# CityU-AIM-Group/SCAN

Measured on AMD Instinct MI355X. Metric: train images/sec (whole node), VGG16 C2F 1024x2048, higher is better.
Workload: dtype f32 (fp32 storage, fp32 multiply, fp32 accumulate -- the reference's arithmetic; the convolutions run it on the bf16 matrix cores as bf16x6: every fp32 operand cut into 3 bf16 pieces = all 24 significand bits, 6 bf16 MFMAs per product)

## Files before the change

### scan_amd/csrc/capi.cpp

```cpp
#include <stdarg.h>
#include <stdio.h>
#include <string.h>

#include "../../include/scan_hip.h"
#include "conv_launch.h"

static thread_local char g_err[512] = "";

extern "C" void scan_set_error(const char* fmt, ...) {
  va_list ap;
  va_start(ap, fmt);
  vsnprintf(g_err, sizeof(g_err), fmt, ap);
  va_end(ap);
}

extern "C" const char* scan_last_error(void) { return g_err; }
extern "C" int scan_abi_version(void) { return 1; }

int g_scan_deterministic = 0;

struct Knob {
  const char* key;
  int* slot;
  int dflt;
};
static Knob* knob_table(int* count) {
  static Knob knobs[] = {
      {"conv_bn256", &g_scan_conv_bn256, 0},   {"conv_v2", &g_scan_conv_v2, 0},         {"conv_wg1024", &g_scan_conv_wg1024, 0},
      {"conv_w8", &g_scan_conv_w8, 0},         {"conv_tpb3", &g_scan_conv_tpb3, 0},     {"conv_bn64_th16", &g_scan_conv_bn64_th16, 0},
      {"conv_glds", &g_scan_conv_glds, 0},     {"wgrad_v6", &g_scan_wgrad_v6, 0},       {"wgrad_prio", &g_scan_wgrad_prio, 0},
      {"wgrad_tile", &g_scan_wgrad_tile, 0},   {"wgrad_wgs", &g_scan_wgrad_wgs, 0},     {"gconv_mfma", &g_scan_gconv_mfma, 0},
      {"dbscan_bf16x3", &g_scan_dbscan_bf16x3, 0}, {"reduce_blocks", &g_scan_reduce_blocks, 0}, {"conv1x1", &g_scan_conv1x1, 0},
      {"conv_wino", &g_scan_conv_wino, 0},     {"wgrad_wino", &g_scan_wgrad_wino, 0},   {"wino_tpb", &g_scan_wino_tpb, 0},
      {"deterministic", &g_scan_deterministic, 0}, {"dynconv_generic", &g_scan_dynconv_generic, 0},
  };
  static bool init = false;
  if (!init) {
    for (auto& k : knobs) k.dflt = *k.slot;
    init = true;
  }
  *count = (int)(sizeof(knobs) / sizeof(knobs[0]));
  return knobs;
}
static Knob* find_knob(const char* key) {
  int n = 0;
  Knob* t = knob_table(&n);
  if (key == nullptr) return nullptr;
  for (int i = 0; i < n; ++i)
    if (strcmp(key, t[i].key) == 0) return &t[i];
  return nullptr;
}

extern "C" int scan_tune(const char* key, int value) {
  Knob* k = find_knob(key);
  if (k == nullptr) return SCAN_TUNE_UNKNOWN;
  const int old = *k->slot;
  *k->slot = value;
  return old;
}

extern "C" int scan_tune_get(const char* key) {
  const Knob* k = find_knob(key);
  return k == nullptr ? SCAN_TUNE_UNKNOWN : *k->slot;
}

extern "C" int scan_tune_default(const char* key) {
  const Knob* k = find_knob(key);
  return k == nullptr ? SCAN_TUNE_UNKNOWN : k->dflt;
}

extern "C" const char* scan_tune_key(int index) {
  int n = 0;
  const Knob* t = knob_table(&n);
  return (index >= 0 && index < n) ? t[index].key : nullptr;
}
```

### scan_amd/csrc/conv_fwd.hip

```cpp
#include "conv_launch.h"
#include "conv_split.h"

#define V2_TW CONV_TILE_W
#ifndef SCAN_CONV_MID
#define SCAN_CONV_MID 0
#endif
#ifndef SCAN_CONV_PFA
#define SCAN_CONV_PFA 1
#endif
#define V2_CK 32

__device__ __forceinline__ int swz(int idx) { return (idx >> 1) & 2; }
__device__ __forceinline__ int wsw(int t, int r) { return ((t >> 1) & 2) ^ (r & 1); }

template <int V>
struct IntC {
  static constexpr int value = V;
};

template <int K>
__device__ __forceinline__ const __bf16* pick_plane(const __bf16* w0, const __bf16* w1, const __bf16* w2) {
  if constexpr (K == 0)
    return w0;
  else if constexpr (K == 1)
    return w1;
  else
    return w2;
}
template <int I, int NT, int PL, int NPL>
__device__ __forceinline__ const __bf16* slot_plane(int tid, const __bf16* w0, const __bf16* w1, const __bf16* w2) {
  constexpr int lo = (NT * I) / PL, hi = (NT * I + NT - 1) / PL;
  constexpr int lo_c = lo < NPL ? lo : NPL - 1, hi_c = hi < NPL ? hi : NPL - 1;
  static_assert(hi - lo <= 1, "a thread's slot spans at most two planes");
  if constexpr (lo_c == hi_c)
    return pick_plane<lo_c>(w0, w1, w2);
  else
    return (tid + NT * I) / PL == lo ? pick_plane<lo_c>(w0, w1, w2) : pick_plane<hi_c>(w0, w1, w2);
}
template <int NT, int PL, int NPL>
__device__ __forceinline__ const __bf16* slot_plane_i(int i, int tid, const __bf16* w0, const __bf16* w1, const __bf16* w2) {
  return i == 0   ? slot_plane<0, NT, PL, NPL>(tid, w0, w1, w2)
         : i == 1 ? slot_plane<1, NT, PL, NPL>(tid, w0, w1, w2)
         : i == 2 ? slot_plane<2, NT, PL, NPL>(tid, w0, w1, w2)
         : i == 3 ? slot_plane<3, NT, PL, NPL>(tid, w0, w1, w2)
         : i == 4 ? slot_plane<4, NT, PL, NPL>(tid, w0, w1, w2)
                  : slot_plane<5, NT, PL, NPL>(tid, w0, w1, w2);
}

template <int NP, int TM, bool TEMP = false>
__device__ __forceinline__ void mma_pieces(const bf16x8 (&w)[NP], const bf16x8 (&p)[NP][TM], f32x4v (&acc)[TM]) {
  if constexpr (TEMP) {
    f32x4v t[TM];
#pragma unroll
    for (int tm = 0; tm < TM; ++tm) t[tm] = f32x4v{0.f, 0.f, 0.f, 0.f};
#pragma unroll
    for (int s = NP - 1; s >= 0; --s)
#pragma unroll
      for (int i = 0; i <= s; ++i)
#pragma unroll
        for (int tm = 0; tm < TM; ++tm) t[tm] = __builtin_amdgcn_mfma_f32_16x16x32_bf16(w[i], p[s - i][tm], t[tm], 0, 0, 0);
#pragma unroll
    for (int tm = 0; tm < TM; ++tm) acc[tm] += t[tm];
    return;
  }
#pragma unroll
  for (int s = NP - 1; s >= 0; --s)
#pragma unroll
    for (int i = 0; i <= s; ++i)
#pragma unroll
      for (int tm = 0; tm < TM; ++tm) acc[tm] = __builtin_amdgcn_mfma_f32_16x16x32_bf16(w[i], p[s - i][tm], acc[tm], 0, 0, 0);
}

__device__ __forceinline__ void gn_sums_add(const float4 o, double& ds, double& dq) {
  const double o0 = (double)o.x, o1 = (double)o.y, o2 = (double)o.z, o3 = (double)o.w;
  ds += (o0 + o1) + (o2 + o3);
  dq += (o0 * o0 + o1 * o1) + (o2 * o2 + o3 * o3);
}

template <int NP, int BN, int TH, int NT, int KS, int TPB = 1, bool GL = false, bool WINO = false>
__global__ __launch_bounds__(NT, NT == 1024 ? 4 : 2) void conv_split_kernel(
    const float* __restrict__ src, scan_pyramid_t d, int Cs, const __bf16* __restrict__ w0, const __bf16* __restrict__ w1,
    const __bf16* __restrict__ w2, int Csw, const float* __restrict__ bias, const float* __restrict__ mask,
    float* __restrict__ dst, int Nout, int Ns, int relu, TileTab2 tt, int n_tiles, scan_pyramid_t sd, int map,
    double* __restrict__ gn_ws) {
  constexpr int HALO = KS / 2, NTAPS = KS * KS;
  constexpr int PH = TH + 2 * HALO;
  constexpr int WJ = WINO ? (TPB == 2 ? 2 : 4) : 1;
  constexpr int PWK = WINO ? WJ * 8 : V2_TW + 2 * HALO;
  constexpr int NPATCH = PH * PWK;
  constexpr int WTAPS = WINO ? 12 : NTAPS;
  constexpr int WAVES = NT / 64;
  constexpr int WN_WAVES = BN >= 128 ? 2 : 1;
  constexpr int WM_WAVES = WAVES / WN_WAVES;
  constexpr int TM = TH / WM_WAVES;
  constexpr int TN = BN / (16 * WN_WAVES);
  constexpr int TMW = WINO ? TM / 2 : TM;
  constexpr int ASLOTS = WINO ? (PH * 64 + NT - 1) / NT : (NPATCH * 8 + NT - 1) / NT;
  constexpr int AK = WINO ? 4 : 1;
  constexpr int BSLOTS = BN * 4 * NP;
  constexpr int BSEG = (BSLOTS + NT - 1) / NT;
  constexpr int NGRP = WTAPS / TPB;
  static_assert(NP == 2 || NP == 3, "two or three pieces per operand");
  static_assert(TM * WM_WAVES == TH && (TM % 2) == 0, "tile rows must split evenly (and pair up for the fused pool)");
  static_assert(WTAPS % TPB == 0, "taps per barrier must divide the tap count");
  static_assert(BSLOTS % 64 == 0, "a wave's 64 weight segments lie in one plane (and past the end only as a whole wave)");
  static_assert(!WINO || (GL && KS == 3 && (TPB == 1 || TPB == 2) && NP == 3 && TM % 2 == 0), "Winograd: three pieces, 3x3, LDS-DMA weights");

  extern __shared__ __align__(16) unsigned char smem_raw[];
  __bf16* As = reinterpret_cast<__bf16*>(smem_raw);
  __bf16* Bs = As + NP * NPATCH * 32;

  const int tid = threadIdx.x, lane = tid & 63, wid = tid >> 6;
  const int bid = xcd_remap(blockIdx.x, gridDim.x);
  const int n_tile = bid % n_tiles;
  const int tile = bid / n_tiles;
  int lvl = 0;
#pragma unroll
  for (int i = 1; i < SCAN_MAX_LEVELS; ++i)
    if (i < d.n_levels && tile >= tt.tile_off[i]) lvl = i;
  const int H = d.h[lvl], W = d.w[lvl];
  int t = tile - tt.tile_off[lvl];
  const int per_img = tt.tiles_x[lvl] * tt.tiles_y[lvl];
  const int img = t / per_img;
  t -= img * per_img;
  const int ty0 = (t / tt.tiles_x[lvl]) * TH, tx0 = (t % tt.tiles_x[lvl]) * V2_TW;
  const int64_t rowbase = d.row_off[lvl] + (int64_t)img * H * W;
  const int n0 = n_tile * BN;
  const int nchunks = (Cs + V2_CK - 1) / V2_CK;

  constexpr unsigned BAD = 0x80000000u;
  unsigned voff[ASLOTS];
  unsigned vok = 0;
  const int c_tail = Cs - (nchunks - 1) * V2_CK;
  const bool tail_bad = 4 * (tid & 7) >= c_tail;
  __amdgpu_buffer_rsrc_t a_src;
  {
    const bool mapped = KS == 1 && map != 0;
    const int Hs = mapped ? sd.h[lvl] : H, Ws = mapped ? sd.w[lvl] : W;
    int64_t base_row;
    if (!mapped)
      base_row = rowbase + (int64_t)(ty0 - HALO) * W + (tx0 - HALO);
    else if (map == 1)
      base_row = sd.row_off[lvl] + ((int64_t)img * Hs + 2 * ty0) * Ws + 2 * tx0;
    else
      base_row = sd.row_off[lvl] + ((int64_t)img * Hs + (ty0 >> 1)) * Ws + (tx0 >> 1);
    a_src = uniform_rsrc_b(src + base_row * Cs, 0x7ffffff0);
    if constexpr (WINO) {
#pragma unroll
      for (int i = 0; i < ASLOTS; ++i) {
        const int slot = tid + NT * i;
        const int c4 = slot & 7, t = (slot >> 3) & 7, py = slot >> 6;
        voff[i] = (unsigned)(((py * W + 2 * t) * Cs + 4 * c4) * 4);
#pragma unroll
        for (int k = 0; k < 4; ++k) {
          const int y = ty0 - HALO + py, x = tx0 - HALO + 2 * t + k;
          if ((slot < PH * 64) && y >= 0 && y < H && x >= 0 && x < W) vok |= 1u << (4 * i + k);
        }
      }
    } else {
#pragma unroll
      for (int i = 0; i < ASLOTS; ++i) {
        const int slot = tid + NT * i;
        const int q = slot >> 3, c4 = slot & 7;
        const int py = q / PWK, px = q - py * PWK;
        const int y = ty0 - HALO + py, x = tx0 - HALO + px;
        bool ok = (slot < NPATCH * 8) && y >= 0 && y < H && x >= 0 && x < W;
        int pix = py * W + px;
        if (mapped) {
          if (map == 1) {
            ok = ok && 2 * y < Hs && 2 * x < Ws;
            pix = 2 * py * Ws + 2 * px;
          } else {
            ok = ok && ((y | x) & 1) == 0 && (y >> 1) < Hs && (x >> 1) < Ws;
            pix = (py >> 1) * Ws + (px >> 1);
          }
        }
        voff[i] = ok ? (unsigned)((pix * Cs + 4 * c4) * 4) : BAD;
      }
    }
  }
  float4 ra[ASLOTS][AK];
  auto load_a = [&](int cc) {
    const int soff = cc * (V2_CK * 4);
    const bool kill = tail_bad && cc == nchunks - 1;
    if constexpr (WINO && TPB == 2) {
      unsigned vk = vok;
      asm volatile("" : "+v"(vk));
#pragma unroll
      for (int i = 0; i < ASLOTS; ++i)
#pragma unroll
        for (int k = 0; k < AK; ++k) {
          const bool ok = ((vk >> (4 * i + k)) & 1) && !kill;
          ra[i][k] = __builtin_bit_cast(float4, __builtin_amdgcn_raw_buffer_load_b128(a_src, (int)(ok ? voff[0] : BAD),
                                                                                      soff + (i * (NT / 64) * W + k) * Cs * 4, 0));
        }
      return;
    }
#pragma unroll
    for (int i = 0; i < ASLOTS; ++i)
#pragma unroll
      for (int k = 0; k < AK; ++k) {
        const unsigned off = !WINO ? voff[i] : ((vok >> (4 * i + k)) & 1) ? voff[i] + (unsigned)(k * Cs * 4) : BAD;
        ra[i][k] = __builtin_bit_cast(float4, __builtin_amdgcn_raw_buffer_load_b128(a_src, (int)(kill ? BAD : off), soff, 0));
      }
  };
  auto store_a = [&](auto half_c) {
    if constexpr (WINO) {
      constexpr int half = decltype(half_c)::value;
#pragma unroll
      for (int i = 0; i < ASLOTS; ++i) {
        const int slot = tid + NT * i;
        if (slot < PH * 64) {
          const int c4 = slot & 7, t = (slot >> 3) & 7, py = slot >> 6;
          const float4 d0 = ra[i][0], d1 = ra[i][1], d2 = ra[i][2], d3 = ra[i][3];
          const float4 u[4] = {make_float4(d0.x - d2.x, d0.y - d2.y, d0.z - d2.z, d0.w - d2.w),
                               make_float4(d1.x + d2.x, d1.y + d2.y, d1.z + d2.z, d1.w + d2.w),
                               make_float4(d2.x - d1.x, d2.y - d1.y, d2.z - d1.z, d2.w - d1.w),
                               make_float4(d1.x - d3.x, d1.y - d3.y, d1.z - d3.z, d1.w - d3.w)};
          const int sl = (((c4 >> 1) ^ wsw(t, py)) << 3) + ((c4 & 1) << 2);
#pragma unroll
          for (int j = 0; j < WJ; ++j) {
            bf16x4 pc[NP];
            split4_np<NP>(u[WJ == 4 ? j : 2 * half + j], pc);
            const int off = (py * PWK + j * 8 + t) * 32 + sl;
#pragma unroll
            for (int p = 0; p < NP; ++p) *reinterpret_cast<bf16x4*>(As + p * NPATCH * 32 + off) = pc[p];
          }
        }
      }
      return;
    }
#pragma unroll
    for (int i = 0; i < ASLOTS; ++i) {
      const int slot = tid + NT * i;
      if (slot < NPATCH * 8) {
        const int q = slot >> 3, c4 = slot & 7;
        const int px = q % PWK;
        bf16x4 pc[NP];
        split4_np<NP>(ra[i][0], pc);
        const int off = q * 32 + (((c4 >> 1) ^ swz(px)) << 3) + ((c4 & 1) << 2);
#pragma unroll
        for (int p = 0; p < NP; ++p) *reinterpret_cast<bf16x4*>(As + p * NPATCH * 32 + off) = pc[p];
      }
    }
  };
  uint4 rb[TPB][BSEG];
  auto load_b = [&](int cc, int grp) {
#pragma unroll
    for (int tt = 0; tt < TPB; ++tt) {
      const int tap = grp * TPB + tt;
#pragma unroll
      for (int i = 0; i < BSEG; ++i) {
        const int slot = tid + NT * i;
        const int plane = slot / (BN * 4);
        const int rem = slot - plane * BN * 4;
        const int row = rem >> 2, seg = rem & 3;
        const int o = n0 + row, c = cc * V2_CK + 8 * seg;
        const __bf16* base = slot_plane_i<NT, BN * 4, NP>(i, tid, w0, w1, w2);
        rb[tt][i] = (slot < BSLOTS && o < Nout && c < Csw)
                        ? *reinterpret_cast<const uint4*>(base + ((int64_t)o * NTAPS + tap) * Csw + c)
                        : make_uint4(0u, 0u, 0u, 0u);
      }
    }
  };
  auto store_b = [&](int buf) {
#pragma unroll
    for (int tt = 0; tt < TPB; ++tt) {
#pragma unroll
      for (int i = 0; i < BSEG; ++i) {
        const int slot = tid + NT * i;
        const int plane = slot / (BN * 4);
        const int rem = slot - plane * BN * 4;
        const int row = rem >> 2, seg = rem & 3;
        if (slot < BSLOTS)
          *reinterpret_cast<uint4*>(Bs + (((buf * TPB + tt) * NP + plane) * BN + row) * 32 + ((seg ^ swz(row)) << 3)) = rb[tt][i];
      }
    }
  };

  static_assert(!GL || BSEG <= 6, "the LDS-DMA path keeps at most six descriptors");
  unsigned boff[BSEG];
#pragma unroll
  for (int i = 0; i < BSEG; ++i) {
    const int slot = tid + NT * i;
    const int plane = slot / (BN * 4);
    const int rem = slot - plane * BN * 4;
    const int row = rem >> 2, seg = (rem & 3) ^ swz(row);
    boff[i] = (unsigned)((((n0 + row) * WTAPS) * Csw + 8 * seg) * 2);
  }
  const int plane_bytes = Nout * WTAPS * Csw * 2;
  auto plane_rsrc = [&](int i) { return uniform_rsrc_b(slot_plane_i<NT, BN * 4, NP>(i, tid, w0, w1, w2), plane_bytes); };
  const __amdgpu_buffer_rsrc_t b_src0 = plane_rsrc(0), b_src1 = plane_rsrc(1), b_src2 = plane_rsrc(2),
                               b_src3 = plane_rsrc(3), b_src4 = plane_rsrc(4), b_src5 = plane_rsrc(5);
  auto issue_b = [&](int cc, int grp, int buf) {
#pragma unroll
    for (int tt = 0; tt < TPB; ++tt) {
      const int tap = grp * TPB + tt;
      const int soff = (tap * Csw + cc * V2_CK) * 2;
#pragma unroll
      for (int i = 0; i < BSEG; ++i) {
        const int slot = tid + NT * i;
        if (BSEG * NT != BSLOTS && slot - lane >= BSLOTS) continue;
        const int plane = slot / (BN * 4);
        const int rem = slot - plane * BN * 4;
        __bf16* dst_l = Bs + (((buf * TPB + tt) * NP + plane) * BN) * 32 + (rem - lane) * 8;
        __builtin_amdgcn_raw_ptr_buffer_load_lds(
            i == 0 ? b_src0 : i == 1 ? b_src1 : i == 2 ? b_src2 : i == 3 ? b_src3 : i == 4 ? b_src4 : b_src5, (lds_ptr_t)dst_l,
            16, (int)boff[i], soff, 0, 0);
      }
    }
  };

  const int wm = wid / WN_WAVES, wn = wid % WN_WAVES;
  const int lr = lane & 15, kg = lane >> 4;
  const int w_row0 = wn * 16 * TN + lr;
  const int w_off = w_row0 * 32 + ((kg ^ swz(w_row0)) << 3);

  f32x4v acc[TN][TM];
#pragma unroll
  for (int b = 0; b < TN; ++b)
#pragma unroll
    for (int a = 0; a < TM; ++a) acc[b][a] = f32x4v{0.f, 0.f, 0.f, 0.f};
  f32x4v wacc[WINO ? 4 : 1][WINO ? TN : 1][TMW];
#pragma unroll
  for (int j = 0; j < (WINO ? 4 : 1); ++j)
#pragma unroll
    for (int b = 0; b < (WINO ? TN : 1); ++b)
#pragma unroll
      for (int a = 0; a < TMW; ++a) wacc[j][b][a] = f32x4v{0.f, 0.f, 0.f, 0.f};

  auto patch_off = [&](int tap) {
    const int ky = tap / KS, kx = tap - KS * ky;
    const int pxs = lr + kx;
    return ((wm * TM + ky) * PWK + pxs) * 32 + ((kg ^ swz(pxs)) << 3);
  };
  auto read_patch = [&](int tap, bf16x8 (&pf)[NP][TM]) {
    const int p_off = patch_off(tap);
#pragma unroll
    for (int p = 0; p < NP; ++p)
#pragma unroll
      for (int tm = 0; tm < TM; ++tm)
        pf[p][tm] = *reinterpret_cast<const bf16x8*>(As + p * NPATCH * 32 + p_off + tm * PWK * 32);
  };
  auto read_w = [&](const __bf16* bt, int tn, bf16x8 (&wf)[NP]) {
#pragma unroll
    for (int p = 0; p < NP; ++p) wf[p] = *reinterpret_cast<const bf16x8*>(bt + p * BN * 32 + tn * 16 * 32);
  };
  auto taps_mma = [&](int grp, int buf, auto&& mid) {
#pragma unroll
    for (int tt = 0; tt < TPB; ++tt) {
      const int tap = grp * TPB + tt;
      const __bf16* bt = Bs + ((buf * TPB + tt) * NP) * BN * 32 + w_off;
      bf16x8 pf[NP][TM];
      read_patch(tap, pf);
#pragma unroll
      for (int tn = 0; tn < TN; ++tn) {
        bf16x8 wf[NP];
        read_w(bt, tn, wf);
        mma_pieces<NP, TM, KS == 1 && NP == 3>(wf, pf, acc[tn]);
        if (tt == 0 && tn == SCAN_CONV_MID) {
          __builtin_amdgcn_sched_barrier(0);
          mid();
          __builtin_amdgcn_sched_barrier(0);
        }
      }
    }
  };
  auto no_mid = []() {};

  constexpr bool PFA = GL && NT == 512 && TPB == 1 && NP == 2 && SCAN_CONV_PFA;
  bf16x8 npf[NP][TM];
  auto taps_mma_pf = [&](int grp, int buf, auto&& mid) {
    if constexpr (PFA) {
      const __bf16* bt = Bs + (buf * NP) * BN * 32 + w_off;
      if (grp == 0) read_patch(0, npf);
#pragma unroll
      for (int tn = 0; tn < TN - 1; ++tn) {
        bf16x8 wf[NP];
        read_w(bt, tn, wf);
        mma_pieces<NP, TM>(wf, npf, acc[tn]);
        if (tn == SCAN_CONV_MID) {
          __builtin_amdgcn_sched_barrier(0);
          mid();
          __builtin_amdgcn_sched_barrier(0);
        }
      }
      {
        constexpr int tn = TN - 1;
        bf16x8 wf[NP];
        read_w(bt, tn, wf);
        const bool more = grp < NGRP - 1;
        const int p_off = patch_off(more ? grp + 1 : grp);
#pragma unroll
        for (int tm = 0; tm < TM; ++tm) {
          acc[tn][tm] = __builtin_amdgcn_mfma_f32_16x16x32_bf16(wf[0], npf[1][tm], acc[tn][tm], 0, 0, 0);
          acc[tn][tm] = __builtin_amdgcn_mfma_f32_16x16x32_bf16(wf[1], npf[0][tm], acc[tn][tm], 0, 0, 0);
          acc[tn][tm] = __builtin_amdgcn_mfma_f32_16x16x32_bf16(wf[0], npf[0][tm], acc[tn][tm], 0, 0, 0);
          npf[0][tm] = *reinterpret_cast<const bf16x8*>(As + p_off + tm * PWK * 32);
          npf[1][tm] = *reinterpret_cast<const bf16x8*>(As + NPATCH * 32 + p_off + tm * PWK * 32);
        }
      }
    }
  };

  auto wino_mma = [&](int j, int ky, int buf, f32x4v (&aj)[WINO ? TN : 1][TMW], auto&& mid, int tt = 0, bool with_mid = true) {
    const __bf16* bt = Bs + ((buf * TPB + tt) * NP) * BN * 32 + w_off;
    const int prow = wm * TM + (lr >> 3) + ky, t = lr & 7;
    const int p_off = (prow * PWK + j * 8 + t) * 32 + ((kg ^ wsw(t, prow)) << 3);
    bf16x8 pf[NP][TMW];
#pragma unroll
    for (int p = 0; p < NP; ++p)
#pragma unroll
      for (int tm = 0; tm < TMW; ++tm)
        pf[p][tm] = *reinterpret_cast<const bf16x8*>(As + p * NPATCH * 32 + p_off + tm * 2 * PWK * 32);
    if constexpr (TPB == 2) {
      bf16x8 wf2[2][NP];
      read_w(bt, 0, wf2[0]);
#pragma unroll
      for (int tn = 0; tn < TN; ++tn) {
        if (tn + 1 < TN) read_w(bt, tn + 1, wf2[(tn + 1) & 1]);
        __builtin_amdgcn_sched_barrier(0);
        mma_pieces<NP, TMW>(wf2[tn & 1], pf, aj[tn]);
        __builtin_amdgcn_sched_barrier(0);
        if (with_mid && tn == 0) {
          mid();
          __builtin_amdgcn_sched_barrier(0);
        }
      }
      return;
    }
#pragma unroll
    for (int tn = 0; tn < TN; ++tn) {
      bf16x8 wf[NP];
      read_w(bt, tn, wf);
      mma_pieces<NP, TMW>(wf, pf, aj[tn]);
      if (with_mid && tn == (SCAN_CONV_MID >= 0 ? SCAN_CONV_MID : 0)) {
        __builtin_amdgcn_sched_barrier(0);
        mid();
        __builtin_amdgcn_sched_barrier(0);
      }
    }
  };

  load_a(0);
  if constexpr (WINO && TPB == 2) {
    issue_b(0, 0, 0);
    for (int cc = 0; cc < nchunks; ++cc) {
      auto ivl = [&](auto g_c, int j0, int ky0, f32x4v (&a0)[WINO ? TN : 1][TMW], int j1, int ky1, f32x4v (&a1)[WINO ? TN : 1][TMW]) {
        constexpr int g = decltype(g_c)::value, buf = g & 1;
        asm volatile("s_waitcnt vmcnt(0)" ::: "memory");
        __syncthreads();
        auto feed = [&]() {
          if (g < NGRP - 1)
            issue_b(cc, g + 1, buf ^ 1);
          else if (cc + 1 < nchunks)
            issue_b(cc + 1, 0, buf ^ 1);
          if (g == NGRP / 2 && cc + 1 < nchunks) load_a(cc + 1);
        };
        wino_mma(j0, ky0, buf, a0, feed, 0, true);
        wino_mma(j1, ky1, buf, a1, no_mid, 1, false);
      };
      auto phase = [&](auto half_c, f32x4v (&a0)[WINO ? TN : 1][TMW], f32x4v (&a1)[WINO ? TN : 1][TMW]) {
        __syncthreads();
        constexpr int half = decltype(half_c)::value;
        store_a(half_c);
        ivl(IntC<3 * half + 0>{}, 0, 0, a0, 0, 1, a0);
        ivl(IntC<3 * half + 1>{}, 0, 2, a0, 1, 0, a1);
        ivl(IntC<3 * half + 2>{}, 1, 1, a1, 1, 2, a1);
      };
      phase(IntC<0>{}, wacc[0], wacc[WINO ? 1 : 0]);
      phase(IntC<1>{}, wacc[WINO ? 2 : 0], wacc[WINO ? 3 : 0]);
    }
  } else if constexpr (WINO) {
    issue_b(0, 0, 0);
    for (int cc = 0; cc < nchunks; ++cc) {
      __syncthreads();
      store_a(IntC<0>{});
      auto comp = [&](int j, f32x4v (&aj)[WINO ? TN : 1][TMW]) {
#pragma unroll 1
        for (int ky = 0; ky < 3; ++ky) {
          const int grp = j * 3 + ky, buf = grp & 1;
          asm volatile("s_waitcnt vmcnt(0)" ::: "memory");
          __syncthreads();
          auto feed = [&]() {
            if (grp < NGRP - 1)
              issue_b(cc, grp + 1, buf ^ 1);
            else if (cc + 1 < nchunks)
              issue_b(cc + 1, 0, buf ^ 1);
            if (grp == NGRP - 2 && cc + 1 < nchunks) load_a(cc + 1);
          };
          wino_mma(j, ky, buf, aj, feed);
        }
      };
      comp(0, wacc[0]);
      comp(1, wacc[WINO ? 1 : 0]);
      comp(2, wacc[WINO ? 2 : 0]);
      comp(3, wacc[WINO ? 3 : 0]);
    }
  } else if constexpr (GL) {
    issue_b(0, 0, 0);
    for (int cc = 0; cc < nchunks; ++cc) {
      __syncthreads();
      store_a(IntC<0>{});
      if (NGRP == 1 && cc + 1 < nchunks) load_a(cc + 1);
#pragma unroll 1
      for (int grp = 0; grp < NGRP; ++grp) {
        const int buf = (cc * NGRP + grp) & 1;
        asm volatile("s_waitcnt vmcnt(0)" ::: "memory");
        __syncthreads();
        auto feed = [&]() {
          if (grp < NGRP - 1)
            issue_b(cc, grp + 1, buf ^ 1);
          else if (cc + 1 < nchunks)
            issue_b(cc + 1, 0, buf ^ 1);
          if (NGRP > 1 && grp == NGRP - 2 && cc + 1 < nchunks) load_a(cc + 1);
        };
        if constexpr (PFA) {
          taps_mma_pf(grp, buf, feed);
        } else if (SCAN_CONV_MID >= 0) {
          taps_mma(grp, buf, feed);
        } else {
          feed();
          taps_mma(grp, buf, no_mid);
        }
      }
    }
  } else {
    load_b(0, 0);
    for (int cc = 0; cc < nchunks; ++cc) {
      __syncthreads();
      store_a(IntC<0>{});
      if (cc + 1 < nchunks) load_a(cc + 1);
#pragma unroll 1
      for (int grp = 0; grp < NGRP; ++grp) {
        const int buf = (cc * NGRP + grp) & 1;
        store_b(buf);
        if (grp < NGRP - 1)
          load_b(cc, grp + 1);
        else if (cc + 1 < nchunks)
          load_b(cc + 1, 0);
        __syncthreads();
        taps_mma(grp, buf, no_mid);
      }
    }
  }

  constexpr bool RELANE = WINO && TPB == 2;
  int tid2 = tid;
  if constexpr (RELANE) asm volatile("" : "+v"(tid2));
  const int etid = RELANE ? tid2 : tid;
  const int ewm = RELANE ? (tid2 >> 6) / WN_WAVES : wm, ewn = RELANE ? (tid2 >> 6) % WN_WAVES : wn;
  const int elr = RELANE ? tid2 & 15 : lr, ekg = RELANE ? (tid2 & 63) >> 4 : kg;
  const int x = tx0 + elr;
  double* gn_red = reinterpret_cast<double*>(smem_raw);
  if (gn_ws != nullptr) __syncthreads();
#pragma unroll
  for (int tn = 0; tn < TN; ++tn) {
    const int o4 = n0 + ewn * 16 * TN + tn * 16 + 4 * ekg;
    float4 bv = make_float4(0.f, 0.f, 0.f, 0.f);
    if (bias != nullptr) {
      bv.x = o4 + 0 < Nout ? bias[o4 + 0] : 0.f;
      bv.y = o4 + 1 < Nout ? bias[o4 + 1] : 0.f;
      bv.z = o4 + 2 < Nout ? bias[o4 + 2] : 0.f;
      bv.w = o4 + 3 < Nout ? bias[o4 + 3] : 0.f;
    }
    if constexpr (WINO) {
      const int xw = tx0 + 2 * (elr & 7);
      if (relu & 2) {
#pragma unroll
        for (int tm = 0; tm < TMW; ++tm) {
          const int y = ty0 + ewm * TM + 2 * tm + (elr >> 3);
          const f32x4v m0 = wacc[0][tn][tm], m1 = wacc[WINO ? 1 : 0][tn][tm], m2 = wacc[WINO ? 2 : 0][tn][tm],
                       m3 = wacc[WINO ? 3 : 0][tn][tm];
          const f32x4v y0 = m0 + (m1 + m2), y1 = (m1 - m2) - m3;
          float v[4];
#pragma unroll
          for (int r = 0; r < 4; ++r) {
            const float m = fmaxf(y0[r], y1[r]);
            v[r] = fmaxf(m, __shfl_xor(m, 8, 64));
          }
          if ((elr >> 3) == 0 && y < H && xw < W && o4 < Nout) {
            const int Hp = H >> 1, Wp = W >> 1;
            float4 o = make_float4(v[0] + bv.x, v[1] + bv.y, v[2] + bv.z, v[3] + bv.w);
            if (relu & 1) {
              o.x = fmaxf(o.x, 0.f);
              o.y = fmaxf(o.y, 0.f);
              o.z = fmaxf(o.z, 0.f);
              o.w = fmaxf(o.w, 0.f);
            }
            *reinterpret_cast<float4*>(dst + ((int64_t)img * Hp * Wp + (int64_t)(y >> 1) * Wp + (xw >> 1)) * Ns + o4) = o;
          }
        }
        continue;
      }
      float4 mk[TMW][2];
      if (mask != nullptr) {
#pragma unroll
        for (int tm = 0; tm < TMW; ++tm) {
          const int y = ty0 + ewm * TM + 2 * tm + (elr >> 3);
#pragma unroll
          for (int e = 0; e < 2; ++e) {
            const bool ok = y < H && xw + e < W && o4 < Nout;
            mk[tm][e] = ok ? *reinterpret_cast<const float4*>(mask + (rowbase + (int64_t)y * W + xw + e) * Ns + o4)
                           : make_float4(0.f, 0.f, 0.f, 0.f);
          }
        }
      }
      double ds = 0.0, dq = 0.0;
#pragma unroll
      for (int tm = 0; tm < TMW; ++tm) {
        const int y = ty0 + ewm * TM + 2 * tm + (elr >> 3);
        const f32x4v m0 = wacc[0][tn][tm], m1 = wacc[WINO ? 1 : 0][tn][tm], m2 = wacc[WINO ? 2 : 0][tn][tm],
                     m3 = wacc[WINO ? 3 : 0][tn][tm];
        const f32x4v yv[2] = {m0 + (m1 + m2), (m1 - m2) - m3};
#pragma unroll
        for (int e = 0; e < 2; ++e) {
          if (y < H && xw + e < W && o4 < Nout) {
            float4 o = make_float4(yv[e][0] + bv.x, yv[e][1] + bv.y, yv[e][2] + bv.z, yv[e][3] + bv.w);
            if (relu & 1) {
              o.x = fmaxf(o.x, 0.f);
              o.y = fmaxf(o.y, 0.f);
              o.z = fmaxf(o.z, 0.f);
              o.w = fmaxf(o.w, 0.f);
            }
            if (mask != nullptr) {
              o.x = (mk[tm][e].x > 0.f) ? o.x : 0.f;
              o.y = (mk[tm][e].y > 0.f) ? o.y : 0.f;
              o.z = (mk[tm][e].z > 0.f) ? o.z : 0.f;
              o.w = (mk[tm][e].w > 0.f) ? o.w : 0.f;
            }
            *reinterpret_cast<float4*>(dst + (rowbase + (int64_t)y * W + xw + e) * Ns + o4) = o;
            if (gn_ws != nullptr) gn_sums_add(o, ds, dq);
          }
        }
      }
      if (gn_ws != nullptr) {
#pragma unroll
        for (int sh = 1; sh <= 16; sh <<= 1) {
          ds += __shfl_xor(ds, sh, 64);
          dq += __shfl_xor(dq, sh, 64);
        }
        if (elr == 0 && (ekg & 1) == 0) {
          double* r = gn_red + (ewm * (BN / 8) + ((o4 - n0) >> 3)) * 2;
          r[0] = ds;
          r[1] = dq;
        }
      }
      continue;
    }
    if (relu & 2) {
      const int Hp = H >> 1, Wp = W >> 1;
#pragma unroll
      for (int tm = 0; tm < TM; tm += 2) {
        const int y = ty0 + ewm * TM + tm;
        float v[4];
#pragma unroll
        for (int r = 0; r < 4; ++r) {
          const float m = fmaxf(acc[tn][tm][r], acc[tn][tm + 1][r]);
          v[r] = fmaxf(m, __shfl_xor(m, 1, 64));
        }
        if ((elr & 1) == 0 && y < H && x < W && o4 < Nout) {
          float4 o = make_float4(v[0] + bv.x, v[1] + bv.y, v[2] + bv.z, v[3] + bv.w);
          if (relu & 1) {
            o.x = fmaxf(o.x, 0.f);
            o.y = fmaxf(o.y, 0.f);
            o.z = fmaxf(o.z, 0.f);
            o.w = fmaxf(o.w, 0.f);
          }
          *reinterpret_cast<float4*>(dst + ((int64_t)img * Hp * Wp + (int64_t)(y >> 1) * Wp + (x >> 1)) * Ns + o4) = o;
        }
      }
      continue;
    }
    float4 mk[TM];
    if (mask != nullptr) {
#pragma unroll
      for (int tm = 0; tm < TM; ++tm) {
        const int y = ty0 + ewm * TM + tm;
        const bool ok = y < H && x < W && o4 < Nout;
        mk[tm] = ok ? *reinterpret_cast<const float4*>(mask + (rowbase + (int64_t)y * W + x) * Ns + o4)
                    : make_float4(0.f, 0.f, 0.f, 0.f);
      }
    }
    double ds = 0.0, dq = 0.0;
#pragma unroll
    for (int tm = 0; tm < TM; ++tm) {
      const int y = ty0 + ewm * TM + tm;
      if (y < H && x < W && o4 < Nout) {
        float4 o = make_float4(acc[tn][tm][0] + bv.x, acc[tn][tm][1] + bv.y, acc[tn][tm][2] + bv.z,
                               acc[tn][tm][3] + bv.w);
        if (relu & 1) {
          o.x = fmaxf(o.x, 0.f);
          o.y = fmaxf(o.y, 0.f);
          o.z = fmaxf(o.z, 0.f);
          o.w = fmaxf(o.w, 0.f);
        }
        if (mask != nullptr) {
          o.x = (mk[tm].x > 0.f) ? o.x : 0.f;
          o.y = (mk[tm].y > 0.f) ? o.y : 0.f;
          o.z = (mk[tm].z > 0.f) ? o.z : 0.f;
          o.w = (mk[tm].w > 0.f) ? o.w : 0.f;
        }
        *reinterpret_cast<float4*>(dst + (rowbase + (int64_t)y * W + x) * Ns + o4) = o;
        if (gn_ws != nullptr) gn_sums_add(o, ds, dq);
      }
    }
    if (gn_ws != nullptr) {
#pragma unroll
      for (int sh = 1; sh <= 16; sh <<= 1) {
        ds += __shfl_xor(ds, sh, 64);
        dq += __shfl_xor(dq, sh, 64);
      }
      if (elr == 0 && (ekg & 1) == 0) {
        double* r = gn_red + (ewm * (BN / 8) + ((o4 - n0) >> 3)) * 2;
        r[0] = ds;
        r[1] = dq;
      }
    }
  }
  if (gn_ws != nullptr) {
    __syncthreads();
    if (etid < BN / 8 * 2) {
      const int g = n0 / 8 + (etid >> 1);
      double v = 0.0;
#pragma unroll
      for (int w = 0; w < WM_WAVES; ++w) v += gn_red[w * (BN / 8) * 2 + etid];
      if (g * 8 < Nout) atomicAdd(&gn_ws[((int64_t)(lvl * d.n_images + img) * 32 + g) * 2 + (etid & 1)], v);
    }
  }
}

template <int NP, int BN, int TH, int NT, int KS, int TPB = 1, bool GL = false, bool WINO = false>
static void launch_v2(const ConvArgs& a) {
  constexpr int HALO = KS / 2;
  TileTab2 tt;
  make_tiles(a.od, &tt, TH);
  const int tiles = tt.tile_off[a.od->n_levels];
  const int n_tiles = (a.Nout + BN - 1) / BN;
  constexpr int PWK = WINO ? (TPB == 2 ? 16 : 32) : V2_TW + 2 * HALO;
  constexpr size_t sh = (size_t)(NP * (TH + 2 * HALO) * PWK * 32 + 2 * NP * TPB * BN * 32) * sizeof(__bf16);
  static_assert(sh <= 160 * 1024, "LDS: 160 KB per CU");
  static bool done = false;
  if (!done) {
    hipFuncSetAttribute(reinterpret_cast<const void*>(conv_split_kernel<NP, BN, TH, NT, KS, TPB, GL, WINO>),
                        hipFuncAttributeMaxDynamicSharedMemorySize, (int)sh);
    done = true;
  }
  hipLaunchKernelGGL((conv_split_kernel<NP, BN, TH, NT, KS, TPB, GL, WINO>), dim3(tiles * n_tiles), dim3(NT), sh, a.st, a.x, *a.od,
                     a.Cs, a.w[0], a.w[1], a.w[2], a.Csw, a.bias, a.mask, a.y, a.Nout, a.Ns, a.relu, tt, n_tiles, *a.sd,
                     a.map, a.gn_ws);
}


static bool wide_tile_costs_no_round(int64_t tiles, int32_t Nout) {
  const int64_t r256 = (tiles * (Nout / 256) + 255) / 256 * 2, r128 = (tiles * (Nout / 128) + 255) / 256;
  return r256 * 97 <= r128 * 100;
}
static int64_t tiles16(const scan_pyramid_t* od) {
  TileTab2 tt;
  make_tiles(od, &tt, 16);
  return tt.tile_off[od->n_levels];
}

int g_scan_conv_bn256 = 2;
int g_scan_conv_wg1024 = 1;
int g_scan_conv_w8 = 1;
int g_scan_conv_tpb3 = 1;
int g_scan_conv_glds = 1;
int g_scan_conv_bn64_th16 = 2;
static int channel_tile3x3(const scan_pyramid_t* od, int32_t Nout) {
  if (Nout <= 64) return 64;
  if (Nout % 256 != 0) return 128;
  const int64_t tiles = tiles16(od);
  if (g_scan_conv_bn256 == 1 && tiles * (Nout / 256) >= 512) return 256;
  if (g_scan_conv_bn256 == 2 && wide_tile_costs_no_round(tiles, Nout)) return 256;
  return 128;
}

#define INST(...) (&launch_v2<__VA_ARGS__>)
ConvInst pick3x3(int np, const scan_pyramid_t* d, int32_t Nout, bool whole_chunks) {
  const int bn = channel_tile3x3(d, Nout);
  const bool gl = g_scan_conv_glds && whole_chunks;
  const bool th16 = g_scan_conv_bn64_th16 && d->n_levels == 1 && d->h[0] % 16 == 0 && d->w[0] % 16 == 0;
  if (np == 3) {
    if (bn == 256) return {256, gl ? INST(3, 256, 16, 512, 3, 1, true) : INST(3, 256, 16, 512, 3)};
    if (bn == 128) return {128, gl ? INST(3, 128, 16, 512, 3, 1, true) : INST(3, 128, 16, 512, 3)};
    if (th16 && g_scan_conv_bn64_th16 == 2 && d->h[0] % 32 == 0)
      return {2064, gl ? INST(3, 64, 32, 512, 3, 1, true) : INST(3, 64, 16, 512, 3)};
    if (th16) return {1064, gl ? INST(3, 64, 16, 512, 3, 1, true) : INST(3, 64, 16, 512, 3)};
    return {64, gl ? INST(3, 64, 8, 256, 3, 1, true) : INST(3, 64, 8, 256, 3)};
  }
  const bool tpb3 = g_scan_conv_tpb3 & 1;
  if (bn == 256) {
    const bool wg16 = g_scan_conv_wg1024 == 1 || (g_scan_conv_wg1024 == 2 && d->n_levels > 1);
    if (g_scan_conv_w8 && g_scan_conv_wg1024 == 1 && gl) return {2256, INST(2, 256, 16, 512, 3, 1, true)};
    if (wg16) return {1256, gl ? INST(2, 256, 16, 1024, 3, 1, true) : INST(2, 256, 16, 1024, 3)};
    return {256, INST(2, 256, 16, 512, 3)};
  }
  if (bn == 128) {
    if (g_scan_conv_wg1024 != 1) return {128, tpb3 ? INST(2, 128, 16, 512, 3, 3) : INST(2, 128, 16, 512, 3)};
    if (gl && Nout % 128 == 0) return {1128, tpb3 ? INST(2, 128, 16, 1024, 3, 3, true) : INST(2, 128, 16, 1024, 3, 1, true)};
    return {1128, tpb3 ? INST(2, 128, 16, 1024, 3, 3) : INST(2, 128, 16, 1024, 3)};
  }
  if (th16) return {64, INST(2, 64, 16, 256, 3)};
  return {64, (g_scan_conv_tpb3 & 2) ? INST(2, 64, 8, 256, 3, 3) : INST(2, 64, 8, 256, 3)};
}

int g_scan_conv1x1 = 3;
ConvInst pick1x1(int np, const scan_pyramid_t* yd, int32_t Nout, int32_t Csw) {
  if (np == 2) return Nout <= 64 ? ConvInst{64, INST(2, 64, 8, 256, 1)} : ConvInst{128, INST(2, 128, 16, 512, 1)};
  if (Nout <= 64) return {64, INST(3, 64, 8, 256, 1)};
  if (!((g_scan_conv1x1 & 1) && Csw % 32 == 0)) return {128, INST(3, 128, 16, 512, 1)};
  if ((g_scan_conv1x1 & 2) && Nout % 256 == 0 && wide_tile_costs_no_round(tiles16(yd), Nout))
    return {1256, INST(3, 256, 16, 512, 1, 1, true)};
  return {1128, INST(3, 128, 16, 512, 1, 1, true)};
}

int g_scan_conv_wino = 1;
int g_scan_wino_tpb = 2;
void conv3x3_wino_launch(const ConvArgs& a) {
  if (g_scan_wino_tpb == 2)
    launch_v2<3, 128, 16, 512, 3, 2, true, true>(a);
  else
    launch_v2<3, 128, 16, 512, 3, 1, true, true>(a);
}
#undef INST
```

### scan_amd/csrc/conv_launch.h

```cpp
#pragma once
#include <hip/hip_runtime_api.h>
#include <stdint.h>

#include "../../include/scan_hip.h"

extern int g_scan_conv_v2;
extern int g_scan_conv_bn256, g_scan_conv_wg1024, g_scan_conv_w8, g_scan_conv_tpb3;
extern int g_scan_conv_glds, g_scan_conv_bn64_th16, g_scan_conv1x1;
extern int g_scan_conv_wino, g_scan_wino_tpb;
extern int g_scan_wgrad_v6, g_scan_wgrad_prio, g_scan_wgrad_tile, g_scan_wgrad_wgs, g_scan_wgrad_wino;
extern int g_scan_gconv_mfma;
extern int g_scan_dynconv_generic;
extern int g_scan_dbscan_bf16x3;
extern int g_scan_reduce_blocks;

struct ConvArgs {
  const float* x;
  const scan_pyramid_t* od;
  const scan_pyramid_t* sd;
  int32_t Cs;
  const __bf16* w[3];
  int32_t Csw;
  const float* bias;
  const float* mask;
  float* y;
  int32_t Nout, Ns, relu, map;
  hipStream_t st;
  double* gn_ws;
};

struct ConvInst {
  int id;
  void (*launch)(const ConvArgs&);
};
ConvInst pick3x3(int np, const scan_pyramid_t* d, int32_t Nout, bool whole_chunks);
ConvInst pick1x1(int np, const scan_pyramid_t* yd, int32_t Nout, int32_t Csw);
void conv3x3_wino_launch(const ConvArgs& a);

void gen1_conv3x3_launch(const ConvArgs& a);
void gen1_conv1x1_launch(const ConvArgs& a);

typedef scan_conv_wgrad_plan_t WgradPlan;
int wgrad_split_plan(const char* name, int np, int ksize, int stride, int32_t Cs, int32_t Cout, const scan_pyramid_t* d, WgradPlan* p);
int wgrad_split_run(const char* name, const WgradPlan& p, const float* x, const scan_pyramid_t* xd, int32_t Cs, const float* dy,
                    const scan_pyramid_t* yd, int32_t Cout, int32_t Cout_s, float* dw, float* db, int32_t accumulate, float* ws,
                    void* stream);
int wgrad_generic_plan(const char* name, int np, int ksize, int stride, int32_t Cs, int32_t Cout, const scan_pyramid_t* yd, WgradPlan* p);
int wgrad_generic_run(const char* name, const WgradPlan& p, const float* x, const scan_pyramid_t* xd, int32_t Cs, const float* dy,
                      const scan_pyramid_t* yd, int32_t Cout, int32_t Cout_s, float* dw, float* db, int32_t accumulate, float* ws,
                      void* stream);
```

Before: 24.99.

## Stage Winograd input transform and LDS stores under the MFMAs in the two-tap conv

Adds a staged variant of the two-tap Winograd forward conv kernel. It splits the activation loads per transform component and interleaves the input transform, bf16 splitting and LDS stores between MFMA groups, using sched_group_barrier. Explicit vmcnt waits replace the full store_a phase barriers, so global loads and LDS writes overlap the matrix work. The variant is enabled by default through a new knob. The cost is more complex scheduling, possible register pressure, and finer-grained wait-count assumptions that could stall the pipeline if they are wrong.

```diff
diff --git a/scan_amd/csrc/capi.cpp b/scan_amd/csrc/capi.cpp
--- a/scan_amd/csrc/capi.cpp
+++ b/scan_amd/csrc/capi.cpp
@@ -33,6 +33,7 @@
       {"dbscan_bf16x3", &g_scan_dbscan_bf16x3, 0}, {"reduce_blocks", &g_scan_reduce_blocks, 0}, {"conv1x1", &g_scan_conv1x1, 0},
       {"conv_wino", &g_scan_conv_wino, 0},     {"wgrad_wino", &g_scan_wgrad_wino, 0},   {"wino_tpb", &g_scan_wino_tpb, 0},
       {"deterministic", &g_scan_deterministic, 0}, {"dynconv_generic", &g_scan_dynconv_generic, 0},
+      {"wino_stage", &g_scan_wino_stage, 0},
   };
   static bool init = false;
   if (!init) {
diff --git a/scan_amd/csrc/conv_fwd.hip b/scan_amd/csrc/conv_fwd.hip
--- a/scan_amd/csrc/conv_fwd.hip
+++ b/scan_amd/csrc/conv_fwd.hip
@@ -7,6 +7,12 @@
 #endif
 #ifndef SCAN_CONV_PFA
 #define SCAN_CONV_PFA 1
+#endif
+#ifndef SCAN_WINO_SPREAD
+#define SCAN_WINO_SPREAD 1
+#endif
+#ifndef SCAN_WINO_VMCNT
+#define SCAN_WINO_VMCNT 1
 #endif
 #define V2_CK 32
 
@@ -77,7 +83,7 @@
   dq += (o0 * o0 + o1 * o1) + (o2 * o2 + o3 * o3);
 }
 
-template <int NP, int BN, int TH, int NT, int KS, int TPB = 1, bool GL = false, bool WINO = false>
+template <int NP, int BN, int TH, int NT, int KS, int TPB = 1, bool GL = false, bool WINO = false, int STG = 0>
 __global__ __launch_bounds__(NT, NT == 1024 ? 4 : 2) void conv_split_kernel(
     const float* __restrict__ src, scan_pyramid_t d, int Cs, const __bf16* __restrict__ w0, const __bf16* __restrict__ w1,
     const __bf16* __restrict__ w2, int Csw, const float* __restrict__ bias, const float* __restrict__ mask,
@@ -105,6 +111,7 @@
   static_assert(WTAPS % TPB == 0, "taps per barrier must divide the tap count");
   static_assert(BSLOTS % 64 == 0, "a wave's 64 weight segments lie in one plane (and past the end only as a whole wave)");
   static_assert(!WINO || (GL && KS == 3 && (TPB == 1 || TPB == 2) && NP == 3 && TM % 2 == 0), "Winograd: three pieces, 3x3, LDS-DMA weights");
+  static_assert(STG == 0 || (WINO && TPB == 2 && ASLOTS == 3 && TN == 4), "staging under the MFMAs: the two-tap Winograd instance");
 
   extern __shared__ __align__(16) unsigned char smem_raw[];
   __bf16* As = reinterpret_cast<__bf16*>(smem_raw);
@@ -180,7 +187,7 @@
     }
   }
   float4 ra[ASLOTS][AK];
-  auto load_a = [&](int cc) {
+  auto load_a = [&](int cc, int km = 15) {
     const int soff = cc * (V2_CK * 4);
     const bool kill = tail_bad && cc == nchunks - 1;
     if constexpr (WINO && TPB == 2) {
@@ -190,6 +197,7 @@
       for (int i = 0; i < ASLOTS; ++i)
 #pragma unroll
         for (int k = 0; k < AK; ++k) {
+          if (!((km >> k) & 1)) continue;
           const bool ok = ((vk >> (4 * i + k)) & 1) && !kill;
           ra[i][k] = __builtin_bit_cast(float4, __builtin_amdgcn_raw_buffer_load_b128(a_src, (int)(ok ? voff[0] : BAD),
                                                                                       soff + (i * (NT / 64) * W + k) * Cs * 4, 0));
@@ -244,6 +252,34 @@
       }
     }
   };
+  int a_base = 0;
+  if constexpr (STG == 1) {
+    const int c4 = tid & 7, t = (tid >> 3) & 7, py = tid >> 6;
+    a_base = (py * PWK + t) * 32 + (((c4 >> 1) ^ wsw(t, py)) << 3) + ((c4 & 1) << 2);
+    static_assert((NT / 64) % 2 == 0, "slots of a thread share the row parity");
+  }
+  auto store_a1 = [&](auto j_c, int i) {
+    constexpr int j = decltype(j_c)::value;
+    if (NT * (i + 1) <= PH * 64 || tid + NT * i < PH * 64) {
+      const float4 &d0 = ra[i][0], &d1 = ra[i][1], &d2 = ra[i][2], &d3 = ra[i][3];
+      float4 u;
+      if constexpr (j == 0) {
+        u = make_float4(d0.x - d2.x, d0.y - d2.y, d0.z - d2.z, d0.w - d2.w);
+      } else if constexpr (j == 1) {
+        u = make_float4(d1.x + d2.x, d1.y + d2.y, d1.z + d2.z, d1.w + d2.w);
+        ra[i][2] = make_float4(d2.x - d1.x, d2.y - d1.y, d2.z - d1.z, d2.w - d1.w);
+      } else if constexpr (j == 2) {
+        u = d2;
+      } else {
+        u = make_float4(d1.x - d3.x, d1.y - d3.y, d1.z - d3.z, d1.w - d3.w);
+      }
+      bf16x4 pc[NP];
+      split4_np<NP>(u, pc);
+      const int off = a_base + (i * (NT / 64) * PWK + (j & 1) * 8) * 32;
+#pragma unroll
+      for (int p = 0; p < NP; ++p) *reinterpret_cast<bf16x4*>(As + p * NPATCH * 32 + off) = pc[p];
+    }
+  };
   uint4 rb[TPB][BSEG];
   auto load_b = [&](int cc, int grp) {
 #pragma unroll
@@ -403,7 +439,8 @@
     }
   };
 
-  auto wino_mma = [&](int j, int ky, int buf, f32x4v (&aj)[WINO ? TN : 1][TMW], auto&& mid, int tt = 0, bool with_mid = true) {
+  auto no_stage = [](int, bool) {};
+  auto wino_mma = [&](int j, int ky, int buf, f32x4v (&aj)[WINO ? TN : 1][TMW], auto&& mid, int tt, bool with_mid, auto&& stage) {
     const __bf16* bt = Bs + ((buf * TPB + tt) * NP) * BN * 32 + w_off;
     const int prow = wm * TM + (lr >> 3) + ky, t = lr & 7;
     const int p_off = (prow * PWK + j * 8 + t) * 32 + ((kg ^ wsw(t, prow)) << 3);
@@ -421,11 +458,13 @@
         if (tn + 1 < TN) read_w(bt, tn + 1, wf2[(tn + 1) & 1]);
         __builtin_amdgcn_sched_barrier(0);
         mma_pieces<NP, TMW>(wf2[tn & 1], pf, aj[tn]);
+        if (with_mid) stage(tn, true);
         __builtin_amdgcn_sched_barrier(0);
         if (with_mid && tn == 0) {
           mid();
           __builtin_amdgcn_sched_barrier(0);
         }
+        if (with_mid) stage(tn, false);
       }
       return;
     }
@@ -442,8 +481,67 @@
     }
   };
 
-  load_a(0);
-  if constexpr (WINO && TPB == 2) {
+  if constexpr (STG != 1) load_a(0);
+  if constexpr (WINO && TPB == 2 && STG == 1) {
+    issue_b(0, 0, 0);
+    load_a(0, 7);
+#pragma unroll
+    for (int i = 0; i < ASLOTS; ++i) store_a1(IntC<0>{}, i);
+    auto chunk = [&](int cc, auto last_c) {
+      constexpr bool last = decltype(last_c)::value != 0;
+      auto ivl = [&](auto g_c, auto sj_c, int j0, int ky0, f32x4v (&a0)[WINO ? TN : 1][TMW], int j1, int ky1,
+                     f32x4v (&a1)[WINO ? TN : 1][TMW]) {
+        constexpr int g = decltype(g_c)::value, buf = g & 1, sj = decltype(sj_c)::value;
+        constexpr bool st = sj > 0 || (sj == 0 && !last);
+        constexpr int pend = !SCAN_WINO_VMCNT ? 0 : (g == 3 || g == 0) ? 3 : (g == 4 && !last) ? 6 : 0;
+        if constexpr (pend == 6) {
+          asm volatile("s_waitcnt vmcnt(6)" ::: "memory");
+        } else if constexpr (pend == 3) {
+          asm volatile("s_waitcnt vmcnt(3)" ::: "memory");
+        } else {
+          asm volatile("s_waitcnt vmcnt(0)" ::: "memory");
+        }
+        __syncthreads();
+        auto feed = [&]() {
+          if (g < NGRP - 1)
+            issue_b(cc, g + 1, buf ^ 1);
+          else if (!last)
+            issue_b(cc + 1, 0, buf ^ 1);
+        };
+        auto stage = [&](int tn, bool inside) {
+          if constexpr (st) {
+            if (inside && (tn == 1 || tn == 2)) {
+              store_a1(sj_c, tn - 1);
+              if (SCAN_WINO_SPREAD)
+#pragma unroll
+              for (int k = 0; k < 12; ++k) {
+                __builtin_amdgcn_sched_group_barrier(0x008, 1, 0);
+                __builtin_amdgcn_sched_group_barrier(0x002, 2, 0);
+                if (k % 4 == 3) __builtin_amdgcn_sched_group_barrier(0x200, 1, 0);
+              }
+            }
+            if (!inside && tn == 2) {
+              store_a1(sj_c, 2);
+              if (sj == 2) load_a(cc, 8);
+              if (sj == 3 && !last) load_a(cc + 1, 5);
+              if (sj == 0) load_a(cc + 1, 2);
+              __builtin_amdgcn_sched_barrier(0);
+            }
+          }
+        };
+        wino_mma(j0, ky0, buf, a0, feed, 0, true, stage);
+        wino_mma(j1, ky1, buf, a1, no_mid, 1, false, no_stage);
+      };
+      ivl(IntC<0>{}, IntC<1>{}, 0, 0, wacc[0], 0, 1, wacc[0]);
+      ivl(IntC<1>{}, IntC<-1>{}, 0, 2, wacc[0], 1, 0, wacc[WINO ? 1 : 0]);
+      ivl(IntC<2>{}, IntC<2>{}, 1, 1, wacc[WINO ? 1 : 0], 1, 2, wacc[WINO ? 1 : 0]);
+      ivl(IntC<3>{}, IntC<3>{}, 0, 0, wacc[WINO ? 2 : 0], 0, 1, wacc[WINO ? 2 : 0]);
+      ivl(IntC<4>{}, IntC<-1>{}, 0, 2, wacc[WINO ? 2 : 0], 1, 0, wacc[WINO ? 3 : 0]);
+      ivl(IntC<5>{}, IntC<0>{}, 1, 1, wacc[WINO ? 3 : 0], 1, 2, wacc[WINO ? 3 : 0]);
+    };
+    for (int cc = 0; cc + 1 < nchunks; ++cc) chunk(cc, IntC<0>{});
+    chunk(nchunks - 1, IntC<1>{});
+  } else if constexpr (WINO && TPB == 2) {
     issue_b(0, 0, 0);
     for (int cc = 0; cc < nchunks; ++cc) {
       auto ivl = [&](auto g_c, int j0, int ky0, f32x4v (&a0)[WINO ? TN : 1][TMW], int j1, int ky1, f32x4v (&a1)[WINO ? TN : 1][TMW]) {
@@ -457,13 +555,19 @@
             issue_b(cc + 1, 0, buf ^ 1);
           if (g == NGRP / 2 && cc + 1 < nchunks) load_a(cc + 1);
         };
-        wino_mma(j0, ky0, buf, a0, feed, 0, true);
-        wino_mma(j1, ky1, buf, a1, no_mid, 1, false);
+        wino_mma(j0, ky0, buf, a0, feed, 0, true, no_stage);
+        wino_mma(j1, ky1, buf, a1, no_mid, 1, false, no_stage);
       };
       auto phase = [&](auto half_c, f32x4v (&a0)[WINO ? TN : 1][TMW], f32x4v (&a1)[WINO ? TN : 1][TMW]) {
         __syncthreads();
         constexpr int half = decltype(half_c)::value;
-        store_a(half_c);
+        if (STG == 2 && cc > 0) {
+#pragma unroll
+          for (int i = 0; i < ASLOTS; ++i)
+#pragma unroll
+            for (int k = 0; k < AK; ++k) asm volatile("" ::"v"(ra[i][k].x), "v"(ra[i][k].y), "v"(ra[i][k].z), "v"(ra[i][k].w));
+        } else
+          store_a(half_c);
         ivl(IntC<3 * half + 0>{}, 0, 0, a0, 0, 1, a0);
         ivl(IntC<3 * half + 1>{}, 0, 2, a0, 1, 0, a1);
         ivl(IntC<3 * half + 2>{}, 1, 1, a1, 1, 2, a1);
@@ -489,7 +593,7 @@
               issue_b(cc + 1, 0, buf ^ 1);
             if (grp == NGRP - 2 && cc + 1 < nchunks) load_a(cc + 1);
           };
-          wino_mma(j, ky, buf, aj, feed);
+          wino_mma(j, ky, buf, aj, feed, 0, true, no_stage);
         }
       };
       comp(0, wacc[0]);
@@ -730,7 +834,7 @@
   }
 }
 
-template <int NP, int BN, int TH, int NT, int KS, int TPB = 1, bool GL = false, bool WINO = false>
+template <int NP, int BN, int TH, int NT, int KS, int TPB = 1, bool GL = false, bool WINO = false, int STG = 0>
 static void launch_v2(const ConvArgs& a) {
   constexpr int HALO = KS / 2;
   TileTab2 tt;
@@ -742,11 +846,11 @@
   static_assert(sh <= 160 * 1024, "LDS: 160 KB per CU");
   static bool done = false;
   if (!done) {
-    hipFuncSetAttribute(reinterpret_cast<const void*>(conv_split_kernel<NP, BN, TH, NT, KS, TPB, GL, WINO>),
+    hipFuncSetAttribute(reinterpret_cast<const void*>(conv_split_kernel<NP, BN, TH, NT, KS, TPB, GL, WINO, STG>),
                         hipFuncAttributeMaxDynamicSharedMemorySize, (int)sh);
     done = true;
   }
-  hipLaunchKernelGGL((conv_split_kernel<NP, BN, TH, NT, KS, TPB, GL, WINO>), dim3(tiles * n_tiles), dim3(NT), sh, a.st, a.x, *a.od,
+  hipLaunchKernelGGL((conv_split_kernel<NP, BN, TH, NT, KS, TPB, GL, WINO, STG>), dim3(tiles * n_tiles), dim3(NT), sh, a.st, a.x, *a.od,
                      a.Cs, a.w[0], a.w[1], a.w[2], a.Csw, a.bias, a.mask, a.y, a.Nout, a.Ns, a.relu, tt, n_tiles, *a.sd,
                      a.map, a.gn_ws);
 }
@@ -818,8 +922,17 @@
 
 int g_scan_conv_wino = 1;
 int g_scan_wino_tpb = 2;
+int g_scan_wino_stage = 1;
+#ifndef SCAN_WINO_STAGE_ABL
+#define SCAN_WINO_STAGE_ABL 0
+#endif
 void conv3x3_wino_launch(const ConvArgs& a) {
-  if (g_scan_wino_tpb == 2)
+#if SCAN_WINO_STAGE_ABL
+  if (g_scan_wino_tpb == 2 && g_scan_wino_stage == 2) return launch_v2<3, 128, 16, 512, 3, 2, true, true, 2>(a);
+#endif
+  if (g_scan_wino_tpb == 2 && g_scan_wino_stage != 0)
+    launch_v2<3, 128, 16, 512, 3, 2, true, true, 1>(a);
+  else if (g_scan_wino_tpb == 2)
     launch_v2<3, 128, 16, 512, 3, 2, true, true>(a);
   else
     launch_v2<3, 128, 16, 512, 3, 1, true, true>(a);
diff --git a/scan_amd/csrc/conv_launch.h b/scan_amd/csrc/conv_launch.h
--- a/scan_amd/csrc/conv_launch.h
+++ b/scan_amd/csrc/conv_launch.h
@@ -7,7 +7,7 @@
 extern int g_scan_conv_v2;
 extern int g_scan_conv_bn256, g_scan_conv_wg1024, g_scan_conv_w8, g_scan_conv_tpb3;
 extern int g_scan_conv_glds, g_scan_conv_bn64_th16, g_scan_conv1x1;
-extern int g_scan_conv_wino, g_scan_wino_tpb;
+extern int g_scan_conv_wino, g_scan_wino_tpb, g_scan_wino_stage;
 extern int g_scan_wgrad_v6, g_scan_wgrad_prio, g_scan_wgrad_tile, g_scan_wgrad_wgs, g_scan_wgrad_wino;
 extern int g_scan_gconv_mfma;
 extern int g_scan_dynconv_generic;
```

Result: no change. 25.30 (median of 3 runs) (+1.3%).
